# phd3/presto-1

Measured on AMD Instinct MI355X. Metric: probe_rows_per_sec, higher is better.
Workload: dtype int64+f64

## Files before the change

### presto-1_amd/__init__.py

```python
from . import _lib, expressions, operators, spi
from ._lib import SO_PATH, TgpuError, build
from .expressions import (and_, between, call, cast, coalesce, constant, field, if_, is_null, not_, or_)
from .operators import (ASC_NULLS_FIRST, ASC_NULLS_LAST, DESC_NULLS_FIRST, DESC_NULLS_LAST, DynamicFilterSourceOperatorFactory, MergePagesOperatorFactory, OrderByOperatorFactory, PartitionedOutputOperator, PartitionedOutputOperatorFactory, TopNOperatorFactory, AVG_BIGINT, AVG_DOUBLE, MIN_BIGINT, MAX_BIGINT, MIN_DOUBLE, MAX_DOUBLE, SUM_ORDER_EXACT, SUM_ORDER_JAVA, COUNT_ALL, COUNT_COLUMN, FINAL, FULL_OUTER, INNER, LOOKUP_OUTER, PARTIAL, PROBE_OUTER, SINGLE, SUM_BIGINT, SUM_DOUBLE,
                        Context, FilterAndProjectOperatorFactory, ScanFilterAndProjectOperatorFactory, PageSource, RecordCursor, FilterProjectHashAggregationOperatorFactory, FilterProjectLookupJoinOperatorFactory, GroupByHash, HashAggregationOperatorFactory, HashBuilderOperatorFactory,
                        LookupJoinOperatorFactory, LookupOuterOperatorFactory, Operator, OperatorFactory, page_processor_source, fused_probe_launch_counts, precompile_fused_aggregation, precompile_fused_probe, precompile_page_processor, to_pages,
                        SET_BITMAP, SET_GENERIC, SET_HASH, HashSemiJoinOperatorFactory, SetBuilderOperatorFactory, SetSupplier,
                        DistinctLimitOperatorFactory, MarkDistinctOperatorFactory,
                        LimitOperatorFactory, RowNumberOperatorFactory,
                        DENSE_RANK, RANK, ROW_NUMBER, TopNRankingOperatorFactory,
                        FRAME_PARTITION, FRAME_RANGE_TO_CURRENT, FRAME_ROWS_TO_CURRENT, WINDOW_AGGREGATE, WINDOW_CUME_DIST, WINDOW_DENSE_RANK, WINDOW_FIRST_VALUE,
                        WINDOW_LAG, WINDOW_LAST_VALUE, WINDOW_LEAD, WINDOW_PERCENT_RANK, WINDOW_RANK, WINDOW_ROW_NUMBER, WindowFunction, WindowOperatorFactory,
                        WINDOW_NTH_VALUE, WINDOW_NTILE, FRAME_TYPE_RANGE, FRAME_TYPE_ROWS, FRAME_TYPE_GROUPS, BOUND_UNBOUNDED_PRECEDING, BOUND_PRECEDING, BOUND_CURRENT_ROW,
                        BOUND_FOLLOWING, BOUND_UNBOUNDED_FOLLOWING, WindowFrame)
from .spi import (BIGINT, BOOLEAN, DATE, DOUBLE, INTEGER, VARCHAR, Block, DeviceBlock, DictionaryBlock, LazyBlock, OutputPage, Page, RunLengthEncodedBlock)
```

### presto-1_amd/_lib.py

```python
import ctypes as C
import os
import subprocess

_HERE = os.path.dirname(os.path.abspath(__file__))
SO_PATH = os.path.join(_HERE, "libtgpu.so")
CSRC = os.path.join(_HERE, "csrc")


class TgpuError(RuntimeError):

    NAMES = {-1: "INVALID_ARGUMENT", -2: "NUMERIC_VALUE_OUT_OF_RANGE", -3: "GENERIC_INSUFFICIENT_RESOURCES", -4: "COMPILER_ERROR",
             -5: "GENERIC_INTERNAL_ERROR", -6: "DEVICE_ERROR", -7: "DIVISION_BY_ZERO", -8: "NOT_SUPPORTED", -9: "INVALID_CAST_ARGUMENT"}

    def __init__(self, code, message):
        super().__init__(f"{self.NAMES.get(code, code)}: {message}")
        self.code = code
        self.message = message


def build(force=False, jobs=8):
    args = ["make", "-C", CSRC, f"-j{jobs}"]
    if force:
        args.append("-B")
    subprocess.check_call(args, stdout=subprocess.DEVNULL)
# ... 66 lines not shown
class WindowFrameSpec(C.Structure):
    _fields_ = [("type", C.c_int32), ("start_type", C.c_int32), ("start_channel", C.c_int32), ("end_type", C.c_int32), ("end_channel", C.c_int32)]


_lib = None

i32, i64, vp, cp = C.c_int32, C.c_int64, C.c_void_p, C.c_char_p
P = C.POINTER
SYMBOLS = {
    "tgpu_context_create": (i32, [i32, vp, P(vp)]),
    "tgpu_context_destroy": (None, [vp]),
    "tgpu_context_synchronize": (i32, [vp]),
    "tgpu_last_error": (cp, []),
    "tgpu_version": (cp, []),
    "tgpu_fused_probe_launch_counts": (i32, [P(i64)]),
    "tgpu_set_resource_dir": (i32, [cp]),
    "tgpu_context_set_double_sum_order": (i32, [vp, i32]),
    "tgpu_context_set_device_input_stable": (i32, [vp, i32]),
    "tgpu_orc_decode_long_column": (i32, [vp, i32, i32, i32, vp, i64, vp, i64, vp]),
    "tgpu_orc_decode_boolean_column": (i32, [vp, i32, vp, i64, vp, i64, vp]),
    "tgpu_orc_decode_dictionary_string_column": (i32, [vp, i32, i32, vp, i64, vp, i64, i32, vp, i64, vp, i64, vp]),
    "tgpu_orc_decode_direct_string_column": (i32, [vp, i32, i32, vp, i64, vp, i64, vp, i64, vp]),
    "tgpu_orc_decode_double_column": (i32, [vp, i32, vp, i64, vp, i64, vp]),
    "tgpu_parquet_decode_data_page": (i32, [vp, i32, i32, i32, i32, vp, i64, vp, i64, vp, i64, i32, vp]),
    "tgpu_context_set_max_output_page": (i32, [vp, i64, i64]),
    "tgpu_pinned_alloc": (i32, [vp, i64, P(vp)]),
    "tgpu_pinned_free": (i32, [vp, vp]),
    "tgpu_profile_enable": (i32, [vp, i32]),
    "tgpu_profile_reset": (i32, [vp]),
    "tgpu_profile_dump": (i64, [vp, cp, i64]),
# ... 118 lines not shown
```

### presto-1_amd/csrc/c_api.cpp

```cpp
#include <atomic>
#include <cstdlib>
#include <map>
#include <mutex>

#include "exchange.h"
#include "kernels.h"
#include "operators.h"
#include "serde.h"
#include "orc.h"
#include "parquet.h"

namespace tgpu {
const std::string &last_error();
}

using namespace tgpu;

namespace {

template <typename F> int32_t guard(F &&f)
{
    try {
        f();
        return TGPU_OK;
// ... 123 lines not shown
int32_t tgpu_context_synchronize(tgpu_context *ctx)
{
    return guard_on(ctx_of(ctx), [&] {
        TG_CHECK_ARG(ctx != nullptr, "context is null");
        ctx->ctx->sync();
    });
}

const char *tgpu_last_error(void) { return last_error().c_str(); }
long long tgpu_debug_bind_count(void) { return g_bind_count.load(); }
const char *tgpu_version(void) { return "tgpu 0.1 (gfx950)"; }
int32_t tgpu_fused_probe_launch_counts(int64_t out[3])
{
    if (!out) return TGPU_ERR_INVALID_ARGUMENT;
    tgpu::fused_probe_launch_counts(out);
    return TGPU_OK;
}

int32_t tgpu_set_resource_dir(const char *dir)
{
    return guard([&] {
        TG_CHECK_ARG(dir != nullptr, "dir is null");
        set_resource_dir(dir);
    });
}

int32_t tgpu_context_set_max_output_page(tgpu_context *ctx, int64_t max_bytes, int64_t max_rows)
{
    return guard_on(ctx_of(ctx), [&] {
        TG_CHECK_ARG(ctx != nullptr && max_bytes >= 0 && max_rows >= 0, "bad argument");
// ... 1320 lines not shown
```

### presto-1_amd/csrc/jit.cpp

```cpp
#include "jit.h"

#include <dlfcn.h>
#include <hip/hiprtc.h>
#include <sys/stat.h>
#include <unistd.h>

#include <algorithm>
#include <fstream>
#include <functional>
#include <list>
#include <tuple>
#include <set>
#include <sstream>

#include "agg.h"
#include "groupby.h"
#include "join.h"
#include "kernels.h"

namespace tgpu {

static std::string g_resource_dir;
static std::mutex g_jit_mu;

// ... 865 lines not shown
    for (int32_t i = 0; i < spec->node_count; i++) {
        const tgpu_expr_node &n = spec->nodes[i];
        put_i32(k, n.kind); put_i32(k, n.type); put_i32(k, n.op); put_i32(k, n.n_args);
        put_i32(k, n.args[0]); put_i32(k, n.args[1]); put_i32(k, n.args[2]); put_i32(k, n.is_null);
        put_i64(k, n.ival);
        k.append(reinterpret_cast<const char *>(&n.dval), 8);
        put_i32(k, n.slen);
    }
    put_i32(k, spec->string_pool_len);
    if (spec->string_pool && spec->string_pool_len > 0) k.append(spec->string_pool, (size_t)spec->string_pool_len);
    put_i32(k, spec->filter_root);
    put_i32(k, spec->projection_count);
    for (int32_t i = 0; i < spec->projection_count; i++) put_i32(k, spec->projection_roots[i]);
    put_i32(k, (int32_t)extra.size());
    for (int32_t v : extra) put_i32(k, v);
    for (const char *env : {"TGPU_FG_EXP", "TGPU_FJ_EXP", "TGPU_FA_STRIPES", "TGPU_FJ_STRIPES", "TGPU_FG_STRIPES"}) {
        const char *v = getenv(env);
        k += '|';
        if (v) k += v;
    }
    return k;
}

template <typename T, typename Make> std::shared_ptr<T> cached_object(const std::string &key, Make make)
{
    static LruCache<T> objects(jit_cache_capacity());
    return objects.get(key, make);
}
}

std::shared_ptr<PageProcessorGpu> PageProcessorGpu::shared(const std::vector<int32_t> &input_types, const tgpu_page_processor_spec *spec)
// ... 152 lines not shown
  void* carry[4];           // FJ_CARRY: block-private regions of the probe-side output VALUES (pass 1 evaluates them from its row
  unsigned char* carry_nulls; // registers for every emitted pair; pass 2 moves them instead of re-reading the input columns sparsely)
  unsigned long long* host_out; // epilogue (small pages): host-visible result words, written by the LAST workgroup of pass 1 (null: none)
  unsigned int* done;           //                         workgroups that have finished (rests at 0)
  const FpArgs* pages;          // FJ_EPILOGUE == 2 (a launch over a LIST of pages): one FpArgs per page, in device memory
  const int* page_tile0;        //   first tile of each page in the launch's tile sequence, [n_pages] = all tiles
  int n_pages;
  int pad3;
};
#define FJ_STRIPES @FJ_STRIPES@
#define FJ_TILE (FJ_STRIPES * 256)
#define FJ_COUNT_SLOTS 64
#ifndef FJ_EPILOGUE
#define FJ_EPILOGUE 0   // the variant for pages (few, one-tile chunks): pass 1 ends with the scan and hands its totals to the host itself
#endif

// rows-capacity offset of block b's private pair region: CHUNKS of 2^chunk_shift consecutive tiles are dealt round-robin, block b
// owns ceil((chunks - b) / grid) of them
__device__ inline long long fj_region_base(long long b, long long tiles, long long grid, int chunk_shift) {
  const long long chunks = (tiles + (1LL << chunk_shift) - 1) >> chunk_shift;
  const long long q = chunks / grid, r = chunks % grid;
  return ((b * q + (b < r ? b : r)) << chunk_shift) * FJ_TILE;
}

@CARRY_FUNCS@
// pass 1: one lane per row.  Matches are compacted in input order inside the tile (ballot + popcount) and appended to the
// block's PRIVATE region, so workgroups never communicate; a scan over the per-tile counts (in tile = input order) then
// gives every tile its final offset and pass 2 moves the pairs there -- probe positions come out ascending exactly as
// LookupJoinPageBuilder.java:144-153 requires.
//
// A probe is a chain of three dependent loads (row -> pre-filter word -> table slot).  The loop is software-pipelined over
// the block's tiles so that the three kinds of load of one iteration belong to three different tiles and are issued back to
// back: iteration `it` issues the row loads of tile it, the pre-filter loads of tile it-1, the slot loads of tile it-2 and
// compacts / writes the pairs of tile it-3, whose slots arrived during the previous iteration.  One memory round trip per
// iteration instead of three (vmcnt is in-order on CDNA: a wait for a dependent load would also wait for every prefetch
// issued before it, so "prefetch, then probe" inside one iteration cannot overlap).
__device__ __forceinline__ void fj_probe_body(const FjArgs& J, const unsigned int bid, const unsigned int nblk) {
  const FpArgs& A = J.fp;
  const int lane = threadIdx.x & 63, w = threadIdx.x >> 6;
  __shared__ int C[2][4];   // pairs of each wave, double-buffered by tile parity (one barrier per tile)
  const long long region = fj_region_base(bid, J.tiles, nblk, J.chunk_shift);
  long long local = 0;      // pairs this block has written so far (uniform across the block)
  unsigned int selected = 0;   // per lane: rows that passed the filter (a lane sees fewer than 2^31 rows)
  // Row layout of a tile: wave w owns the contiguous rows [w * 64 * FJ_STRIPES, (w + 1) * 64 * FJ_STRIPES) of the tile and its
  // lane reads row s * 64 + lane of them in stripe s (512 contiguous bytes per wave and load).  Input order inside the tile is
  // then (wave, stripe, lane): the compaction needs the other waves' TOTALS only, everything else is wave-local scalar work.
  // Rows are 32-bit here (a page has fewer than 2^31 positions).
#if FJ_EPILOGUE != 2
  const unsigned int n_rows = (unsigned int)A.n;
#endif
  const unsigned int wave_row = (unsigned int)w * (64u * FJ_STRIPES) + (unsigned int)lane;
// ... 14 lines not shown
  // the descriptor of the page stage A will load from is fetched ONE ITERATION AHEAD (scalar loads: the search of the tile's page and the
  // page's column pointers are two dependent round trips that would otherwise sit in front of every iteration's row loads)
  int pN = 0;
  long long tN = 0;   // tile of the next iteration's stage A (my_tiles == 0: unused)
  {
    const long long t0 = tile_of(0);
    tN = (my_tiles > 0 && t0 < J.tiles) ? t0 : 0;
    while (tN >= (long long)pt0[pN + 1]) pN++;
  }
  FpArgs AN = pgs[pN];    // next stage A's page
  FpArgs AB = AN;         // this iteration's stage B page (= the previous iteration's stage A page)
  long long tB0 = 0;      // first tile of that page
  long long tN0 = pt0[pN];
#endif
  long long chunk_local0 = 0;   // `local` at the start of the chunk being compacted
  TgRow rw[FJ_STRIPES];                                                                                            // stage A -> B
  long long pkey[FJ_STRIPES]; unsigned int psidx[FJ_STRIPES]; unsigned long long pbw[FJ_STRIPES];                      // B -> C
#if FJ_PF == 2
  unsigned long long pbits[FJ_STRIPES];     // Bloom mask of the key
#else
  unsigned int pbits[FJ_STRIPES];           // bit of the key inside its bitmap word
#endif
  unsigned char pfl[FJ_STRIPES];                                                                                   // 1 = probe, 2 = passed the filter
#if FJ_PF == 1 || FJ_PF == 3
  const unsigned long long key_range = (unsigned long long)J.pf.key_max - (unsigned long long)J.pf.key_min;
#endif
  long long skey[FJ_STRIPES]; unsigned int ssidx[FJ_STRIPES]; unsigned char sfl[FJ_STRIPES]; TgSlot16 ssl[FJ_STRIPES]; // C -> D
#if FJ_CARRY
  TgOut pov[FJ_STRIPES], sov[FJ_STRIPES];   // the row's output values, travelling B -> C -> D with its key
#pragma unroll
  for (int s = 0; s < FJ_STRIPES; s++) { tg_zero_out(pov[s]); tg_zero_out(sov[s]); }
#endif
#if FJ_CARRY == 2
  // PARTIAL carry: only outputs that the filter / key row already holds travel (no load, no TgRow field is added), and stage D keeps
  // its place behind the loads -- the values of tile jD step aside (dov) before stage C takes the stage registers for tile jC
  TgOut dov[FJ_STRIPES];
#pragma unroll
  for (int s = 0; s < FJ_STRIPES; s++) tg_zero_out(dov[s]);
#endif
#pragma unroll
  for (int s = 0; s < FJ_STRIPES; s++) {
    tg_zero_row(rw[s]);
    pkey[s] = 0; psidx[s] = 0; pbits[s] = 0; pbw[s] = 0; pfl[s] = 0;
    skey[s] = 0; ssidx[s] = 0; sfl[s] = 0; ssl[s].key = 0; ssl[s].head = -1; ssl[s].count = 0;
  }
  for (long long it = 0; it < my_tiles + 3; it++) {
    const long long jD = it - 3, jC = it - 2, jB = it - 1, jA = it;
    __builtin_amdgcn_s_waitcnt(0x0F70);   // vmcnt(0): everything the previous iteration issued (consumed right below anyway)
    // stage D, part 1: resolve tile jD from the slots loaded by the previous iteration; only a collision with another key
    // walks further
    int head[FJ_STRIPES];
    bool emit[FJ_STRIPES];
#pragma unroll
    for (int s = 0; s < FJ_STRIPES; s++) { head[s] = -1; emit[s] = false; }
    const bool doD = jD >= 0 && tile_of(jD) < J.tiles;
    if (doD) {
#pragma unroll
      for (int s = 0; s < FJ_STRIPES; s++) {
#if FJ_PF == 3
        // the bitmap is exact: the key is in the build side.  The pair carries the key's rank among the build keys (present keys
        // in front of its bitmap word, loaded by the previous iteration, + set bits below its own); fj_emit reads the build
        // position at that rank, for the matching rows only
        // (nobody reads the build positions: the rank structure may not even be built -- rank_base[0] is then whatever the buffer held)
// ... 110 lines not shown
#pragma unroll
    for (int s = 0; s < FJ_STRIPES; s++) bidx[s] = 0;
    if (doB) {
#if FJ_EPILOGUE == 2
      const unsigned int n_rows = (unsigned int)AB.n;
      const unsigned int row0 = (unsigned int)((tile_of(jB) - tB0) * FJ_TILE) + wave_row;   // the page's own rows
#else
      const FpArgs& AB = A;
      const unsigned int row0 = (unsigned int)(tile_of(jB) * FJ_TILE) + wave_row;
#endif
#pragma unroll
      for (int s = 0; s < FJ_STRIPES; s++) {
        const unsigned int row = row0 + s * 64;
        bool sel = false, passed = false;
        long long key = 0;
        if (row < n_rows && tg_filter(AB, row, rw[s])) {
          selected++;
          passed = true;
          const bool kn = tg_key(AB, row, rw[s], key);   // JoinProbe.java:87-97: a null probe key never matches
          sel = !kn;
#if FJ_CARRY
          tg_carry_eval(AB, row, rw[s], pov[s]);
#endif
        }
        bidx[s] = 0;
#if FJ_PF == 1 || FJ_PF == 3
        {
          // key in [key_min, key_max] <=> (key - key_min) mod 2^64 <= key_max - key_min; a key outside cannot match: no probe
          const unsigned long long d = (unsigned long long)key - (unsigned long long)J.pf.key_min;
          sel = sel && d <= key_range;
          pbits[s] = (unsigned int)d & 63u;
          bidx[s] = sel ? (unsigned int)(d >> 6) : 0u;
        }
#elif FJ_PF == 2
        {
          const unsigned long long hm = tg_fmix64((unsigned long long)tg_hash_long(key));
          pbits[s] = tg_bloom_mask(hm);
// ... 21 lines not shown
      ssl[s].head = J.pf.rank_base[cidx[s]];   // DIRECT layout: present keys in front of the survivor's bitmap word (entry 0 otherwise: unused)
#else
      ssl[s] = J.slots[cidx[s]];
#endif
    }
#pragma unroll
    for (int s = 0; s < FJ_STRIPES; s++) {
#if FJ_PF == 1 || FJ_PF == 3
      pbw[s] = J.pf.bitmap[bidx[s]];
#elif FJ_PF == 2
      pbw[s] = J.pf.bloom[bidx[s]];
#else
      pbw[s] = ~0ULL;
#endif
    }
    {
#if FJ_EPILOGUE == 2
      // this iteration's page was fetched by the previous one (idle stage: the same page again, its first tile)
      const FpArgs AA = AN;
      const long long tA = doA ? tN : tN0;
      const unsigned int n_rows = (unsigned int)AA.n;
      const unsigned int tile_row0 = (unsigned int)((tA - tN0) * FJ_TILE);
      const unsigned int row0 = tile_row0 + wave_row;
      AB = AA;      // (stage B of the NEXT iteration works on the rows loaded here; this iteration's stage B has run already)
      tB0 = tN0;
      {             // and the page of the next iteration's tile: issued now, needed in an iteration's time
        const long long jn = jA + 1;
        if (jn < my_tiles && tile_of(jn) < J.tiles) {
          tN = tile_of(jn);
          while (tN >= (long long)pt0[pN + 1]) pN++;
          tN0 = pt0[pN];
          AN = pgs[pN];
        }
      }
#else
      const FpArgs& AA = A;
      const unsigned int row0 = (unsigned int)((doA ? tile_of(jA) : 0LL) * FJ_TILE) + wave_row;
      const unsigned int tile_row0 = (unsigned int)((doA ? tile_of(jA) : 0LL) * FJ_TILE);
#endif
      if (tile_row0 + FJ_TILE <= n_rows) {   // interior tile: one address per column, the stripes are constant offsets from it
#pragma unroll
        for (int s = 0; s < FJ_STRIPES; s++) tg_load_row(AA, row0 + s * 64, rw[s]);
      }
      else {
#pragma unroll
        for (int s = 0; s < FJ_STRIPES; s++) {
          const unsigned int row = row0 + s * 64;
          tg_load_row(AA, row < n_rows ? row : n_rows - 1, rw[s]);
        }
      }
    }
    __builtin_amdgcn_sched_barrier(0);
#if FJ_CARRY != 1
    // stage D, part 2: compact the pairs of tile jD in input order and append them to the block's region
    if (doD) {
      const long long tile = tile_of(jD);
      const unsigned int row0 = (unsigned int)(tile * FJ_TILE) + wave_row;
      if ((jD & cmask) == 0) chunk_local0 = local;
      unsigned long long b[FJ_STRIPES];
      int wave_total = 0;
#pragma unroll
      for (int s = 0; s < FJ_STRIPES; s++) {
        b[s] = __ballot(emit[s]);
        wave_total += __popcll(b[s]);
      }
      int* Cw = C[jD & 1];
      if (lane == 0) Cw[w] = wave_total;
// ... 16 lines not shown
        }
        o += (unsigned int)__popcll(b[s]);
      }
      local += tile_total;
      // per-chunk bookkeeping, rewritten after every tile of the chunk (the last one stands)
      if (threadIdx.x == 0) {
#if FJ_EPILOGUE   // (agent-scope store: the epilogue's reader may sit on another XCD)
        __hip_atomic_store(&J.tile_cnt[tile >> csh], (int)(local - chunk_local0), __ATOMIC_RELAXED, __HIP_MEMORY_SCOPE_AGENT);
#else
        J.tile_cnt[tile >> csh] = (int)(local - chunk_local0);
#endif
        J.tile_src[tile >> csh] = (int)chunk_local0;
      }
    }
#endif
  }
  // rows that passed the filter: ONE atomic per workgroup, spread over FJ_COUNT_SLOTS words on separate cache lines (the host adds
  unsigned long long selected_wave = selected;
#pragma unroll
  for (int d = 32; d >= 1; d >>= 1) selected_wave += __shfl_down(selected_wave, d, 64);
  __shared__ unsigned long long S[4];
  if (lane == 0) S[w] = selected_wave;
  __syncthreads();
#if !FJ_EPILOGUE
  if (threadIdx.x == 0) {
    const unsigned long long block_total = S[0] + S[1] + S[2] + S[3];
    if (block_total) atomicAdd(&J.counters[(bid % FJ_COUNT_SLOTS) * 16], block_total);
  }
}
#else
  // Epilogue of a small page (J.host_out): the workgroup that finishes LAST scans the chunk counts into the chunks' output offsets (what
// ... 180 lines not shown
        if (nd.kind == TGPU_EX_CALL || nd.kind == TGPU_EX_SPECIAL)
            for (int k = 0; k < nd.n_args; k++)
                if (can_raise(nd.args[k])) return true;
        return false;
    };
    for (size_t ch = 0; ch < proj_roots_.size(); ch++)
        if ((int)ch != join_channel_ && can_raise(proj_roots_[ch])) supported_ = false;
    key_can_raise_ = can_raise(proj_roots_[(size_t)join_channel_]);
    if (supported_) generate();
}

FusedProbeGpu::~FusedProbeGpu() {}

static std::atomic<int64_t> g_fj_launches[3];
constexpr int kFjFreeRule = 1;
void fused_probe_launch_counts(int64_t out[3])
{
    for (int i = 0; i < 3; i++) out[i] = g_fj_launches[i].load(std::memory_order_relaxed);
}

void FusedProbeGpu::generate()
{
    auto cols_decl = [&](const Gen &g) {
        std::ostringstream cols;
        for (int ch : g.used_cols) {
            const int32_t t = input_types_[(size_t)ch];
            const char *T = (t == TGPU_VARCHAR || t == TGPU_BOOLEAN) ? "unsigned char" : ctype(t);
            cols << "  const " << T << "* c" << ch << " = (const " << T << "*)A.col_values[" << ch << "]; (void)c" << ch << ";\n";
            cols << "  const unsigned char* cn" << ch << " = FJ_NO_NULLS ? (const unsigned char*)0 : A.col_nulls[" << ch << "]; (void)cn" << ch << ";\n";
            if (t == TGPU_VARCHAR) cols << "  const int* co" << ch << " = A.col_offsets[" << ch << "]; (void)co" << ch << ";\n";
        }
        return cols.str();
    };
// ... 92 lines not shown
    src << "#if FJ_CARRY\n";
    for (int ch : carry_only_cols) src << field(ch);
    src << "#endif\n";
    if (gr.reg_cols.empty()) src << "  int unused;\n";
    src << "};\n__device__ inline void tg_load_row(const FpArgs& A, long long row, TgRow& R) {\n";
    for (int ch : gr.reg_cols) src << load(ch);
    src << "#if FJ_CARRY\n";
    for (int ch : carry_only_cols) src << load(ch);
    src << "#endif\n";
    src << "  (void)A; (void)row; (void)R;\n}\n__device__ inline void tg_zero_row(TgRow& R) {\n";
    for (int ch : gr.reg_cols) src << "  R.c" << ch << " = 0; R.n" << ch << " = 0;\n";
    src << "#if FJ_CARRY\n";
    for (int ch : carry_only_cols) src << "  R.c" << ch << " = 0; R.n" << ch << " = 0;\n";
    src << "#endif\n";
    src << "  (void)R;\n}\n";
    const std::string rc = cols_decl(gr), mc = cols_decl(gm);
    for (auto &b : reg_bodies) src << splice(b, rc);
    for (auto &b : mem_bodies) src << splice(b, mc);
    src << "struct FjArgs;\nstruct TgOut {\n";
    for (size_t i = 0; i < output_channels_.size(); i++) src << all_or_free(i) << "  " << ctype(proj_types_[(size_t)output_channels_[i]]) << " v" << i << ";\n#endif\n";
    src << "#if !FJ_NO_NULLS\n  unsigned char nulls;\n#endif\n};\n__device__ inline void tg_zero_out(TgOut& O) {\n";
    for (size_t i = 0; i < output_channels_.size(); i++) src << all_or_free(i) << "  O.v" << i << " = 0;\n#endif\n";
    src << "#if !FJ_NO_NULLS\n  O.nulls = 0;\n#endif\n  (void)O;\n}\n#if FJ_CARRY\n";
    {
        const std::string cc = cols_decl(gc);
        for (size_t i = 0; i < carry_bodies.size(); i++) src << all_or_free(i) << splice(carry_bodies[i], cc) << "#endif\n";
        src << "__device__ inline void tg_carry_eval(const FpArgs& A, long long row, const TgRow& R, TgOut& O) {\n  unsigned char nl = 0;\n";
        for (size_t i = 0; i < output_channels_.size(); i++) {
            const int32_t t = proj_types_[(size_t)output_channels_[i]];
            src << all_or_free(i) << "  { " << ctype(t) << " v = 0; const bool n = tg_c" << i << "(A, row, R, v); O.v" << i << " = n ? (" << ctype(t) << ")0 : v; nl |= n ? " << (1 << i)
// ... 19 lines not shown
                    << "]) A.out_nulls[" << i << "][to] = (unsigned char)((nl >> " << i << ") & 1u);\n#endif\n";
    }
    carry_funcs << "}\n#endif\n";
    (void)kt;
    src << "__device__ inline void tg_emit_outputs(const FpArgs& A, long long row, long long o) {\n  (void)A; (void)row; (void)o;\n";
    for (size_t i = 0; i < output_channels_.size(); i++) {
        const int ch = output_channels_[i];
        const int32_t t = proj_types_[(size_t)ch];
        const char *T = t == TGPU_BOOLEAN ? "unsigned char" : ctype(t);
        src << not_carried(i) << "  { " << ctype(t) << " v = 0; const bool n = tg_p" << ch << "(A, row, v); ((" << T << "*)A.out_values[" << i << "])[o] = n ? (" << T << ")0 : (" << T
            << ")v; if (A.out_nulls[" << i << "]) A.out_nulls[" << i << "][o] = n ? 1 : 0; }\n#endif\n";
    }
    src << "}\n";
    if (const char *exp = getenv("TGPU_FJ_EXP")) src << "#define FJ_EXP_" << exp << " 1\n";
    {
        std::string kernels = kFjKernels;
        const std::string tag = "@FJ_STRIPES@";
        kernels.replace(kernels.find(tag), tag.size(), std::to_string(fj_stripes()));
        const std::string ctag = "@CARRY_FUNCS@";
        kernels.replace(kernels.find(ctag), ctag.size(), carry_funcs.str());
        src << kernels;
    }
    source_ = src.str();
}

static std::string prefilter_source(const std::string &src, int variant)
{
    static const char *layout[4] = {"plain", "bitmap", "bloom", "direct"};
    const std::string l = layout[variant % 4];
    return "#define FJ_PF " + std::to_string(variant % 4) + "\n#define FJ_NO_NULLS " + std::to_string((variant / 4) % 2) + "\n#define FJ_CARRY " + std::to_string(variant / 24) +
           "\n#define FJ_EPILOGUE " + std::to_string((variant / 8) % 3) + "\n#define fj_pair fj_pair_" + l + "\n#define fj_probe fj_probe_" + l +
           "\n#define fj_emit fj_emit_" + l + "\n" + src;
}

void FusedProbeGpu::precompile()
{
    if (!supported_) return;
    for (int variant = 0; variant < 24; variant++) {
        (void)code_object_for(prefilter_source(source_, variant));
        if (partial_supported_ && (variant % 4 == 1 || variant % 4 == 3) && variant / 8 < 2) (void)code_object_for(prefilter_source(source_, 48 + variant));
    }
}

JitModule *FusedProbeGpu::module_for(int kind, bool no_nulls, int carry, int epilogue)
{
    std::lock_guard<std::mutex> lk(mu_);
    const int variant = kind + (no_nulls ? 4 : 0) + epilogue * 8 + carry * 24;
    if (!modules_[variant]) modules_[variant] = load_module(prefilter_source(source_, variant));
    return modules_[variant].get();
}

struct FusedProbeGpu::Pending {
    FjArgs J{};
    JitModule *module = nullptr;
    int pf_kind = 0;
    int64_t chunks = 0;
    bool outer = false, need_build_positions = false;
    int carry = 0;
    BufferPtr tile_cnt, tile_src, tile_dst, misc, pair_probe, pair_build;
    std::vector<BufferPtr> carry_regions;
    Context::AsyncRead read;
    Context::Signal signal;
// ... 47 lines not shown
    int64_t n = in.n;
    if (multi) {
        int64_t t = 0;
        for (const DevicePage *pg : pages) {
            TG_CHECK_ARG(pg->n > 0, "empty page in a multi-page launch");
            page_tile0.push_back((int32_t)t);
            t += ceil_div(pg->n, tile_rows);
        }
        page_tile0.push_back((int32_t)t);
        TG_CHECK_ARG(t <= kFjMultiMaxTiles, "too many rows for one multi-page launch");
        n = t * tile_rows;
        carry = 0;
    }
    if (n == 0) return nullptr;
    const bool page_variant = multi || (ceil_div(n, tile_rows) <= kFjEpilogueMaxChunks && getenv("TGPU_DISABLE_PROBE_EPILOGUE") == nullptr);
    JitModule *module = module_for(tv.rank_base ? 3 : (tv.bitmap ? 1 : (tv.bloom ? 2 : 0)), !any_nulls, carry, multi ? 2 : (page_variant ? 1 : 0));
    std::shared_ptr<Pending> pend = std::make_shared<Pending>();
    pend->col_nulls = col_nulls;
    pend->kernel_variant = multi ? 2 : (page_variant ? 1 : 0);
    if (page_variant) pend->signal = ctx->begin_signal();
    if (multi && pend->signal.slot < 0) return nullptr;
    struct SignalGuard {
        Context *ctx;
        Context::Signal *signal;
        bool armed = true;
        ~SignalGuard()
        {
            if (armed && signal->slot >= 0) {
                ctx->abandon_signal(*signal);
                signal->slot = -1;
            }
// ... 12 lines not shown
    J.fp.n = multi ? in.n : n;
    J.slots = tv.slots;
    J.mask = tv.mask;
    J.bitmap = tv.bitmap;
    J.key_min = tv.key_min;
    J.key_max = tv.key_max;
    J.bloom = tv.bloom;
    J.bloom_word_mask = tv.bloom_word_mask;
    J.direct = tv.direct;
    J.rank_base = tv.rank_base;
    J.outer = (outer ? 1 : 0) | (need_build_positions ? 0 : 2);
    J.tiles = ceil_div(n, tile_rows);
    TG_CHECK_ARG(n <= 0x7fffffffLL && J.tiles <= 0x7fffffffLL, "page too large");
    const int pf_kind = tv.rank_base ? 3 : (tv.bitmap ? 1 : (tv.bloom ? 2 : 0));
    static const char *probe_names[4] = {"fj_probe_plain", "fj_probe_bitmap", "fj_probe_bloom", "fj_probe_direct"};
    const int64_t resident = (int64_t)ctx->cu_count() * module->blocks_per_cu(probe_names[pf_kind]);
    int chunk_shift = 0;
    const int max_chunk_shift = getenv("TGPU_FJ_CHUNK_SHIFT") ? atoi(getenv("TGPU_FJ_CHUNK_SHIFT")) : 6;
    while (!multi && chunk_shift < max_chunk_shift && (J.tiles >> (chunk_shift + 1)) >= 4 * resident) chunk_shift++;
    J.chunk_shift = chunk_shift;
    const int64_t chunks = (J.tiles + (1ll << chunk_shift) - 1) >> chunk_shift;
    pend->chunks = chunks;
    pend->pf_kind = pf_kind;
    const int64_t grid1 = std::min<int64_t>(chunks, resident);
    J.grid1 = grid1;
    BufferPtr tile_cnt = ctx->alloc((size_t)chunks * 4), tile_src = ctx->alloc((size_t)chunks * 4), tile_dst = ctx->alloc((size_t)chunks * 4);
    constexpr int kMiscWords = kFjMiscWords;
    static_assert((size_t)kFjMiscWords * 8 <= Context::kZeroedScratchBytes, "the probe's counters fit the context's scratch words");
    if (pend->signal.slot >= 0 && chunk_shift != 0) {
        ctx->abandon_signal(pend->signal);
        pend->signal.slot = -1;
// ... 46 lines not shown
        for (size_t i = 0; i < output_channels_.size(); i++) {
            if (carry == 2 && !free_out_[i]) continue;
            carry_regions.push_back(ctx->alloc((size_t)cap * type_width(proj_types_[(size_t)output_channels_[i]])));
            J.carry[i] = carry_regions.back()->ptr();
            const tgpu_expr_node &root = nodes_[(size_t)proj_roots_[(size_t)output_channels_[i]]];
            nullable = nullable || !(root.kind == TGPU_EX_INPUT && root.op >= 0 && root.op < (int)in.cols.size() && in.cols[(size_t)root.op].nulls == nullptr);
        }
        if (nullable) {
            carry_regions.push_back(ctx->alloc((size_t)cap));
            J.carry_nulls = carry_regions.back()->as<uint8_t>();
        }
    }
    pend->grid1 = grid1;
    pend->tile_cnt = tile_cnt; pend->tile_src = tile_src; pend->tile_dst = tile_dst; pend->misc = misc; pend->pair_probe = pair_probe; pend->pair_build = pair_build;
    g_fj_launches[carry].fetch_add(1, std::memory_order_relaxed);
    if (launch || !epilogue) launch_probe(ctx, pend);
    signal_guard.armed = false;
    return pend;
}

void FusedProbeGpu::launch_probe(Context *ctx, const std::shared_ptr<Pending> &pend)
{
    static const char *probe_names[4] = {"fj_probe_plain", "fj_probe_bitmap", "fj_probe_bloom", "fj_probe_direct"};
    if (!pend || pend->probe_launched) return;
    FjArgs &J = pend->J;
    {
        ProfileScope ps(ctx, "fused_filter_probe");
        launch_args(pend->module->fn(probe_names[pend->pf_kind]), (int)pend->grid1, J, ctx->stream());
    }
    pend->probe_launched = true;
// ... 1481 lines not shown
```

### presto-1_amd/csrc/jit.h

```cpp
#pragma once

#include <algorithm>

#include "common.h"

namespace tgpu {

constexpr int kFpMaxCols = 24;
constexpr int kFpMaxProj = 16;

struct FpArgs {
    const void *col_values[kFpMaxCols];
    const uint8_t *col_nulls[kFpMaxCols];
    const int32_t *col_offsets[kFpMaxCols];
    void *out_values[kFpMaxProj];
    uint8_t *out_nulls[kFpMaxProj];
    int32_t *positions;
    const int32_t *tile_offsets;
    int32_t *tile_counts;
    unsigned long long *error;
    long long n;
    unsigned long long *sel_mask;
};

// ... 83 lines not shown
    void *carry[4];
    uint8_t *carry_nulls;
    unsigned long long *host_out;
    unsigned int *done;
    const FpArgs *pages;
    const int32_t *page_tile0;
    int32_t n_pages;
    int32_t pad3;
};
constexpr int kFjMaxBuildCols = 4;
constexpr int64_t kFjMultiMaxTiles = 32768;
constexpr int64_t kFjEpilogueMaxChunks = 2048;

class LookupSourceGpu;
void fused_probe_launch_counts(int64_t out[3]);

class FusedProbeGpu {
public:
    FusedProbeGpu(std::vector<int32_t> input_types, const tgpu_page_processor_spec *spec, int32_t join_channel, std::vector<int32_t> output_channels);
    ~FusedProbeGpu();
    static std::shared_ptr<FusedProbeGpu> shared(const std::vector<int32_t> &input_types, const tgpu_page_processor_spec *spec, int32_t join_channel,
                                                 const std::vector<int32_t> &output_channels);
    void precompile();
    bool supported() const { return supported_; }
    const std::vector<int32_t> &projection_types() const { return proj_types_; }
    void process(Context *ctx, const DevicePage &in, const LookupSourceGpu &source, bool outer, bool need_build_positions, std::vector<DeviceColumn> &probe_out,
                 BufferPtr &build_idx, int64_t &count, int64_t &selected_rows, const std::vector<DeviceColumn> *build_cols = nullptr,
                 std::vector<DeviceColumn> *build_out = nullptr);
    struct Pending;
    std::shared_ptr<Pending> begin(Context *ctx, const DevicePage &in, const LookupSourceGpu &source, bool outer, bool need_build_positions, bool launch = true);
    std::shared_ptr<Pending> begin(Context *ctx, const std::vector<const DevicePage *> &pages, const LookupSourceGpu &source, bool outer, bool need_build_positions,
                                   bool launch = true);
    static int64_t multi_page_row_limit();
    void finish(Context *ctx, const std::shared_ptr<Pending> &pending, const DevicePage &in, std::vector<DeviceColumn> &probe_out, BufferPtr &build_idx, int64_t &count,
                int64_t &selected_rows, const std::vector<DeviceColumn> *build_cols = nullptr, std::vector<DeviceColumn> *build_out = nullptr, bool launch = true);
    void launch_probe(Context *ctx, const std::shared_ptr<Pending> &pending);
    void launch_emit(Context *ctx, const std::shared_ptr<Pending> &pending);
    bool can_pair(const std::shared_ptr<Pending> &emit_side, const std::shared_ptr<Pending> &probe_side) const;
    void launch_pair(Context *ctx, const std::shared_ptr<Pending> &emit_side, const std::shared_ptr<Pending> &probe_side);
    void cancel(Context *ctx, const std::shared_ptr<Pending> &pending);
    const std::string &source() const { return source_; }

private:
    void generate();
    struct JitModule *module_for(int prefilter_kind, bool no_nulls, int carry, int epilogue);
    std::mutex mu_;
    std::vector<int32_t> input_types_;
    std::vector<tgpu_expr_node> nodes_;
    std::string pool_;
    int filter_root_;
    std::vector<int32_t> proj_roots_, proj_types_, output_channels_;
    int32_t join_channel_;
    bool supported_ = false;
    std::string source_;
    std::shared_ptr<JitModule> modules_[72];
    bool carry_supported_ = false;
    bool partial_supported_ = false, key_can_raise_ = false;
    std::vector<bool> free_out_;
};

class GroupedAccumulators;

class FusedAggGpu {
public:
    FusedAggGpu(std::vector<int32_t> input_types, const tgpu_page_processor_spec *spec, std::vector<tgpu_agg_spec> aggs,
                std::vector<int32_t> group_by_channels = {});
    static std::shared_ptr<FusedAggGpu> shared(const std::vector<int32_t> &input_types, const tgpu_page_processor_spec *spec,
                                               const std::vector<tgpu_agg_spec> &aggs, const std::vector<int32_t> &group_by_channels);
    const std::vector<int> &key_inputs() const { return key_inputs_; }
    void probe_groups(Context *ctx, const DevicePage &in, const struct GbhProbeLaunch &l);
// ... 51 lines not shown
```

### presto-1_amd/operators.py

```python
import ctypes as C
import json

import numpy as np

from . import _lib
from .expressions import FlatProgram
from .spi import OutputPage, Page

COUNT_ALL, COUNT_COLUMN, SUM_BIGINT, SUM_DOUBLE, AVG_BIGINT, AVG_DOUBLE, MIN_BIGINT, MAX_BIGINT, MIN_DOUBLE, MAX_DOUBLE = 1, 2, 3, 4, 5, 6, 7, 8, 9, 10
SINGLE, PARTIAL, FINAL = 0, 1, 2
ASC_NULLS_FIRST, ASC_NULLS_LAST, DESC_NULLS_FIRST, DESC_NULLS_LAST = 0, 1, 2, 3
INNER, PROBE_OUTER, LOOKUP_OUTER, FULL_OUTER = 0, 1, 2, 3
SUM_ORDER_EXACT, SUM_ORDER_JAVA = 0, 1


def _i32(seq):
    seq = list(seq)
    return (C.c_int32 * max(1, len(seq)))(*seq), len(seq)


class Context:

    def __init__(self, device=0, stream=None):
        h = C.c_void_p()
# ... 501 lines not shown
    gc, ng = _i32(group_by_channels)
    _lib.check(_lib.lib().tgpu_precompile_fused_aggregation(nt, t, C.byref(spec), len(aggs), arr, ng, gc))


def precompile_fused_probe(input_types, filter_expr, projections, join_channel, probe_output_channels):
    prog = FlatProgram(filter_expr, projections)
    spec, keep = prog.to_c()
    t, nt = _i32(input_types)
    oc, no = _i32(probe_output_channels)
    _lib.check(_lib.lib().tgpu_precompile_fused_probe(nt, t, C.byref(spec), join_channel, no, oc))


def fused_probe_launch_counts():
    out = (C.c_int64 * 3)()
    _lib.check(_lib.lib().tgpu_fused_probe_launch_counts(out))
    return tuple(int(v) for v in out)


class GroupByHash:

    def __init__(self, ctx: Context, types, hash_channels, input_hash_channel=None, expected_size=100):
        t, n = _i32(types)
        hc, _ = _i32(hash_channels)
        h = C.c_void_p()
        _lib.check(_lib.lib().tgpu_group_by_hash_create(ctx.handle, n, t, hc, -1 if input_hash_channel is None else input_hash_channel,
                                                        expected_size, C.byref(h)))
        self.handle = h

    def addPage(self, page: Page):
        cp, keep = page.to_c()
# ... 339 lines not shown
```

Before: 88.21 billion.

## Add depth-2 row prefetch to fused probe kernel with partial vmcnt wait

Adds a second set of row registers to the whole-table fused join probe kernel so the rows of the next tile are loaded while the current iteration waits for hash look-ups. The loop body is emitted twice per trip with alternating register sets, and the top-of-iteration wait leaves the youngest row loads outstanding using a computed vmcnt. Depth 2 is the default for carry modes 0 and 2 on whole-table launches, and it doubles the module variant table. In exchange it raises register pressure, which may lower occupancy, and increases JIT compile variants. Also adds depth launch counters and an env cap on resident blocks.

```diff
diff --git a/presto-1_amd/__init__.py b/presto-1_amd/__init__.py
--- a/presto-1_amd/__init__.py
+++ b/presto-1_amd/__init__.py
@@ -3,7 +3,7 @@
 from .expressions import (and_, between, call, cast, coalesce, constant, field, if_, is_null, not_, or_)
 from .operators import (ASC_NULLS_FIRST, ASC_NULLS_LAST, DESC_NULLS_FIRST, DESC_NULLS_LAST, DynamicFilterSourceOperatorFactory, MergePagesOperatorFactory, OrderByOperatorFactory, PartitionedOutputOperator, PartitionedOutputOperatorFactory, TopNOperatorFactory, AVG_BIGINT, AVG_DOUBLE, MIN_BIGINT, MAX_BIGINT, MIN_DOUBLE, MAX_DOUBLE, SUM_ORDER_EXACT, SUM_ORDER_JAVA, COUNT_ALL, COUNT_COLUMN, FINAL, FULL_OUTER, INNER, LOOKUP_OUTER, PARTIAL, PROBE_OUTER, SINGLE, SUM_BIGINT, SUM_DOUBLE,
                         Context, FilterAndProjectOperatorFactory, ScanFilterAndProjectOperatorFactory, PageSource, RecordCursor, FilterProjectHashAggregationOperatorFactory, FilterProjectLookupJoinOperatorFactory, GroupByHash, HashAggregationOperatorFactory, HashBuilderOperatorFactory,
-                        LookupJoinOperatorFactory, LookupOuterOperatorFactory, Operator, OperatorFactory, page_processor_source, fused_probe_launch_counts, precompile_fused_aggregation, precompile_fused_probe, precompile_page_processor, to_pages,
+                        LookupJoinOperatorFactory, LookupOuterOperatorFactory, Operator, OperatorFactory, page_processor_source, fused_probe_launch_counts, fused_probe_depth_counts, precompile_fused_aggregation, precompile_fused_probe, precompile_page_processor, to_pages,
                         SET_BITMAP, SET_GENERIC, SET_HASH, HashSemiJoinOperatorFactory, SetBuilderOperatorFactory, SetSupplier,
                         DistinctLimitOperatorFactory, MarkDistinctOperatorFactory,
                         LimitOperatorFactory, RowNumberOperatorFactory,
diff --git a/presto-1_amd/_lib.py b/presto-1_amd/_lib.py
--- a/presto-1_amd/_lib.py
+++ b/presto-1_amd/_lib.py
@@ -104,6 +104,7 @@
     "tgpu_last_error": (cp, []),
     "tgpu_version": (cp, []),
     "tgpu_fused_probe_launch_counts": (i32, [P(i64)]),
+    "tgpu_fused_probe_depth_counts": (i32, [P(i64)]),
     "tgpu_set_resource_dir": (i32, [cp]),
     "tgpu_context_set_double_sum_order": (i32, [vp, i32]),
     "tgpu_context_set_device_input_stable": (i32, [vp, i32]),
diff --git a/presto-1_amd/csrc/c_api.cpp b/presto-1_amd/csrc/c_api.cpp
--- a/presto-1_amd/csrc/c_api.cpp
+++ b/presto-1_amd/csrc/c_api.cpp
@@ -161,6 +161,12 @@
 {
     if (!out) return TGPU_ERR_INVALID_ARGUMENT;
     tgpu::fused_probe_launch_counts(out);
+    return TGPU_OK;
+}
+int32_t tgpu_fused_probe_depth_counts(int64_t out[2])
+{
+    if (!out) return TGPU_ERR_INVALID_ARGUMENT;
+    tgpu::fused_probe_depth_counts(out);
     return TGPU_OK;
 }
 
diff --git a/presto-1_amd/csrc/jit.cpp b/presto-1_amd/csrc/jit.cpp
--- a/presto-1_amd/csrc/jit.cpp
+++ b/presto-1_amd/csrc/jit.cpp
@@ -903,7 +903,7 @@
     for (int32_t i = 0; i < spec->projection_count; i++) put_i32(k, spec->projection_roots[i]);
     put_i32(k, (int32_t)extra.size());
     for (int32_t v : extra) put_i32(k, v);
-    for (const char *env : {"TGPU_FG_EXP", "TGPU_FJ_EXP", "TGPU_FA_STRIPES", "TGPU_FJ_STRIPES", "TGPU_FG_STRIPES"}) {
+    for (const char *env : {"TGPU_FG_EXP", "TGPU_FJ_EXP", "TGPU_FA_STRIPES", "TGPU_FJ_STRIPES", "TGPU_FG_STRIPES", "TGPU_FJ_DEPTH"}) {
         const char *v = getenv(env);
         k += '|';
         if (v) k += v;
@@ -1086,6 +1086,22 @@
 #ifndef FJ_EPILOGUE
 #define FJ_EPILOGUE 0   // the variant for pages (few, one-tile chunks): pass 1 ends with the scan and hands its totals to the host itself
 #endif
+#ifndef FJ_DEPTH
+#define FJ_DEPTH 1      // row sets in flight: 2 = the rows of the tile after next are loaded while this iteration's look-ups are waited for
+#endif
+#if FJ_DEPTH == 2 && FJ_EPILOGUE
+#error "FJ_DEPTH 2 is a variant of the whole-table kernel only"
+#endif
+#if FJ_DEPTH == 2
+// The iteration's wait leaves the youngest row set outstanding: vmcnt counts loads AND stores on this target and retires them in order,
+// so the row loads are the last vector-memory operations an iteration issues (behind the pair stores).  FJ_ROW_LOADS = load instructions
+// per row as generated; the count is 6 bits wide, [3:0] and [15:14] of the operand (0x0F70: no wait on the other counters).  Correctness
+// does not rest on the number: the compiler adds whatever wait a register use needs.
+#define FJ_PENDING (FJ_ROW_LOADS * FJ_STRIPES > 63 ? 63 : FJ_ROW_LOADS * FJ_STRIPES)
+#define FJ_WAIT (0x0F70 | (FJ_PENDING & 15) | ((FJ_PENDING >> 4) << 14))
+#else
+#define FJ_WAIT 0x0F70  // vmcnt(0): everything the previous iteration issued (consumed right below anyway)
+#endif
 
 // rows-capacity offset of block b's private pair region: CHUNKS of 2^chunk_shift consecutive tiles are dealt round-robin, block b
 // owns ceil((chunks - b) / grid) of them
@@ -1107,6 +1123,12 @@
 // compacts / writes the pairs of tile it-3, whose slots arrived during the previous iteration.  One memory round trip per
 // iteration instead of three (vmcnt is in-order on CDNA: a wait for a dependent load would also wait for every prefetch
 // issued before it, so "prefetch, then probe" inside one iteration cannot overlap).
+//
+// FJ_DEPTH 2 (whole-table launches): a second set of row registers.  Iteration `it` issues the rows of tile it+1 -- as its LAST
+// vector-memory operations, behind the pair stores -- and waits at its top for everything but that youngest set, so a wave always has a
+// tile's rows in flight, also while it waits for its look-ups.  Stage B of iteration `it` consumes the set issued by iteration it-2 (tile
+// it-1; the prologue issues tile 0).  The two sets alternate by writing the loop body twice per trip, never by copying registers (a copy
+// from a register with a pending load waits for the load).  Rows per lane, compaction order and pairs are those of depth 1.
 __device__ __forceinline__ void fj_probe_body(const FjArgs& J, const unsigned int bid, const unsigned int nblk) {
   const FpArgs& A = J.fp;
   const int lane = threadIdx.x & 63, w = threadIdx.x >> 6;
@@ -1151,7 +1173,11 @@
   long long tN0 = pt0[pN];
 #endif
   long long chunk_local0 = 0;   // `local` at the start of the chunk being compacted
+#if FJ_DEPTH == 2
+  TgRow rwa[FJ_STRIPES], rwb[FJ_STRIPES];                                                                          // stage A -> B: tiles of even / odd j
+#else
   TgRow rw[FJ_STRIPES];                                                                                            // stage A -> B
+#endif
   long long pkey[FJ_STRIPES]; unsigned int psidx[FJ_STRIPES]; unsigned long long pbw[FJ_STRIPES];                      // B -> C
 #if FJ_PF == 2
   unsigned long long pbits[FJ_STRIPES];     // Bloom mask of the key
@@ -1177,13 +1203,27 @@
 #endif
 #pragma unroll
   for (int s = 0; s < FJ_STRIPES; s++) {
+#if FJ_DEPTH == 2
+    tg_zero_row(rwa[s]); tg_zero_row(rwb[s]);
+#else
     tg_zero_row(rw[s]);
+#endif
     pkey[s] = 0; psidx[s] = 0; pbits[s] = 0; pbw[s] = 0; pfl[s] = 0;
     skey[s] = 0; ssidx[s] = 0; sfl[s] = 0; ssl[s].key = 0; ssl[s].head = -1; ssl[s].count = 0;
   }
-  for (long long it = 0; it < my_tiles + 3; it++) {
-    const long long jD = it - 3, jC = it - 2, jB = it - 1, jA = it;
-    __builtin_amdgcn_s_waitcnt(0x0F70);   // vmcnt(0): everything the previous iteration issued (consumed right below anyway)
+#if FJ_DEPTH == 2
+  // whole trips of two iterations: an exit between the two instances of the body would be one more way into the loop header for the compiler's
+  // wait-count bookkeeping, with the other row set pending there.  The odd iteration out is idle (every tile at or past my_tiles is past J.tiles).
+  const long long n_it = (my_tiles + 4) & ~1LL;
+#else
+  const long long n_it = my_tiles + 3;
+#endif
+@FJ_LOOP@
+)SRC";
+
+const char *kFjLoopBody = R"SRC(
+    const long long jD = it - 3, jC = it - 2, jB = it - 1, jA = it + (FJ_DEPTH - 1);
+    __builtin_amdgcn_s_waitcnt(FJ_WAIT);
     // stage D, part 1: resolve tile jD from the slots loaded by the previous iteration; only a collision with another key
     // walks further
     int head[FJ_STRIPES];
@@ -1324,13 +1364,13 @@
         const unsigned int row = row0 + s * 64;
         bool sel = false, passed = false;
         long long key = 0;
-        if (row < n_rows && tg_filter(AB, row, rw[s])) {
+        if (row < n_rows && tg_filter(AB, row, @RW@[s])) {
           selected++;
           passed = true;
-          const bool kn = tg_key(AB, row, rw[s], key);   // JoinProbe.java:87-97: a null probe key never matches
+          const bool kn = tg_key(AB, row, @RW@[s], key);   // JoinProbe.java:87-97: a null probe key never matches
           sel = !kn;
 #if FJ_CARRY
-          tg_carry_eval(AB, row, rw[s], pov[s]);
+          tg_carry_eval(AB, row, @RW@[s], pov[s]);
 #endif
         }
         bidx[s] = 0;
@@ -1382,6 +1422,20 @@
       pbw[s] = ~0ULL;
 #endif
     }
+#if FJ_DEPTH != 2
+@ROW_LOADS@
+#endif
+    __builtin_amdgcn_sched_barrier(0);
+@STAGE_D2@
+#if FJ_DEPTH == 2
+    // the rows of tile jA = it + 1: the youngest vector-memory operations of the iteration, behind stage D's stores (see FJ_WAIT)
+    __builtin_amdgcn_sched_barrier(0);
+@ROW_LOADS@
+    __builtin_amdgcn_sched_barrier(0);
+#endif
+)SRC";
+
+const char *kFjRowLoads = R"SRC(
     {
 #if FJ_EPILOGUE == 2
       // this iteration's page was fetched by the previous one (idle stage: the same page again, its first tile)
@@ -1408,17 +1462,19 @@
 #endif
       if (tile_row0 + FJ_TILE <= n_rows) {   // interior tile: one address per column, the stripes are constant offsets from it
 #pragma unroll
-        for (int s = 0; s < FJ_STRIPES; s++) tg_load_row(AA, row0 + s * 64, rw[s]);
+        for (int s = 0; s < FJ_STRIPES; s++) tg_load_row(AA, row0 + s * 64, @RW@[s]);
       }
       else {
 #pragma unroll
         for (int s = 0; s < FJ_STRIPES; s++) {
           const unsigned int row = row0 + s * 64;
-          tg_load_row(AA, row < n_rows ? row : n_rows - 1, rw[s]);
+          tg_load_row(AA, row < n_rows ? row : n_rows - 1, @RW@[s]);
         }
       }
     }
-    __builtin_amdgcn_sched_barrier(0);
+)SRC";
+
+const char *kFjStageD2 = R"SRC(
 #if FJ_CARRY != 1
     // stage D, part 2: compact the pairs of tile jD in input order and append them to the block's region
     if (doD) {
@@ -1465,7 +1521,9 @@
       }
     }
 #endif
-  }
+)SRC";
+
+const char *kFjKernelsTail = R"SRC(
   // rows that passed the filter: ONE atomic per workgroup, spread over FJ_COUNT_SLOTS words on separate cache lines (the host adds
   unsigned long long selected_wave = selected;
 #pragma unroll
@@ -1676,9 +1734,21 @@
 
 static std::atomic<int64_t> g_fj_launches[3];
 constexpr int kFjFreeRule = 1;
+static std::atomic<int64_t> g_fj_depth_launches[2];
+constexpr int kFjDepthByCarry[3] = {2, 1, 2};
+static int fj_depth_for(int carry, int epilogue)
+{
+    if (epilogue != 0) return 1;
+    if (const char *e = getenv("TGPU_FJ_DEPTH")) return atoi(e) == 2 ? 2 : 1;
+    return kFjDepthByCarry[carry];
+}
 void fused_probe_launch_counts(int64_t out[3])
 {
     for (int i = 0; i < 3; i++) out[i] = g_fj_launches[i].load(std::memory_order_relaxed);
+}
+void fused_probe_depth_counts(int64_t out[2])
+{
+    for (int i = 0; i < 2; i++) out[i] = g_fj_depth_launches[i].load(std::memory_order_relaxed);
 }
 
 void FusedProbeGpu::generate()
@@ -1801,6 +1871,7 @@
     for (int ch : carry_only_cols) src << "  R.c" << ch << " = 0; R.n" << ch << " = 0;\n";
     src << "#endif\n";
     src << "  (void)R;\n}\n";
+    src << "#define FJ_ROW_LOADS ((" << gr.reg_cols.size() << " + (FJ_CARRY == 1 ? " << carry_only_cols.size() << " : 0)) * (FJ_NO_NULLS ? 1 : 2))\n";
     const std::string rc = cols_decl(gr), mc = cols_decl(gm);
     for (auto &b : reg_bodies) src << splice(b, rc);
     for (auto &b : mem_bodies) src << splice(b, mc);
@@ -1850,7 +1921,16 @@
     src << "}\n";
     if (const char *exp = getenv("TGPU_FJ_EXP")) src << "#define FJ_EXP_" << exp << " 1\n";
     {
-        std::string kernels = kFjKernels;
+        auto replace_all = [](std::string t, const std::string &tag, const std::string &with) {
+            for (size_t p = t.find(tag); p != std::string::npos; p = t.find(tag, p + with.size())) t.replace(p, tag.size(), with);
+            return t;
+        };
+        const std::string body = replace_all(replace_all(kFjLoopBody, "@STAGE_D2@", kFjStageD2), "@ROW_LOADS@", kFjRowLoads);
+        const std::string loop = std::string("#if FJ_DEPTH == 2\n  {\n    const long long jA = 0;\n    const bool doA = jA < my_tiles && tile_of(jA) < J.tiles;\n") +
+                                 replace_all(kFjRowLoads, "@RW@", "rwa") + "  }\n  for (long long it = 0; it < n_it;) {\n    {\n" + replace_all(body, "@RW@", "rwb") +
+                                 "    }\n    ++it;\n    {\n" + replace_all(body, "@RW@", "rwa") + "    }\n    ++it;\n  }\n#else\n" +
+                                 "  for (long long it = 0; it < n_it; it++) {\n" + replace_all(body, "@RW@", "rw") + "  }\n#endif\n";
+        std::string kernels = replace_all(kFjKernels, "@FJ_LOOP@", loop) + kFjKernelsTail;
         const std::string tag = "@FJ_STRIPES@";
         kernels.replace(kernels.find(tag), tag.size(), std::to_string(fj_stripes()));
         const std::string ctag = "@CARRY_FUNCS@";
@@ -1864,8 +1944,8 @@
 {
     static const char *layout[4] = {"plain", "bitmap", "bloom", "direct"};
     const std::string l = layout[variant % 4];
-    return "#define FJ_PF " + std::to_string(variant % 4) + "\n#define FJ_NO_NULLS " + std::to_string((variant / 4) % 2) + "\n#define FJ_CARRY " + std::to_string(variant / 24) +
-           "\n#define FJ_EPILOGUE " + std::to_string((variant / 8) % 3) + "\n#define fj_pair fj_pair_" + l + "\n#define fj_probe fj_probe_" + l +
+    return "#define FJ_PF " + std::to_string(variant % 4) + "\n#define FJ_NO_NULLS " + std::to_string((variant / 4) % 2) + "\n#define FJ_CARRY " + std::to_string((variant / 24) % 3) +
+           "\n#define FJ_DEPTH " + std::to_string(variant / 72 + 1) + "\n#define FJ_EPILOGUE " + std::to_string((variant / 8) % 3) + "\n#define fj_pair fj_pair_" + l + "\n#define fj_probe fj_probe_" + l +
            "\n#define fj_emit fj_emit_" + l + "\n" + src;
 }
 
@@ -1873,15 +1953,17 @@
 {
     if (!supported_) return;
     for (int variant = 0; variant < 24; variant++) {
-        (void)code_object_for(prefilter_source(source_, variant));
-        if (partial_supported_ && (variant % 4 == 1 || variant % 4 == 3) && variant / 8 < 2) (void)code_object_for(prefilter_source(source_, 48 + variant));
-    }
-}
-
-JitModule *FusedProbeGpu::module_for(int kind, bool no_nulls, int carry, int epilogue)
+        const int epilogue = variant / 8;
+        (void)code_object_for(prefilter_source(source_, variant + 72 * (fj_depth_for(0, epilogue) - 1)));
+        if (partial_supported_ && (variant % 4 == 1 || variant % 4 == 3) && epilogue < 2)
+            (void)code_object_for(prefilter_source(source_, 48 + variant + 72 * (fj_depth_for(2, epilogue) - 1)));
+    }
+}
+
+JitModule *FusedProbeGpu::module_for(int kind, bool no_nulls, int carry, int epilogue, int depth)
 {
     std::lock_guard<std::mutex> lk(mu_);
-    const int variant = kind + (no_nulls ? 4 : 0) + epilogue * 8 + carry * 24;
+    const int variant = kind + (no_nulls ? 4 : 0) + epilogue * 8 + carry * 24 + (depth - 1) * 72;
     if (!modules_[variant]) modules_[variant] = load_module(prefilter_source(source_, variant));
     return modules_[variant].get();
 }
@@ -1959,7 +2041,8 @@
     }
     if (n == 0) return nullptr;
     const bool page_variant = multi || (ceil_div(n, tile_rows) <= kFjEpilogueMaxChunks && getenv("TGPU_DISABLE_PROBE_EPILOGUE") == nullptr);
-    JitModule *module = module_for(tv.rank_base ? 3 : (tv.bitmap ? 1 : (tv.bloom ? 2 : 0)), !any_nulls, carry, multi ? 2 : (page_variant ? 1 : 0));
+    const int depth = fj_depth_for(carry, multi ? 2 : (page_variant ? 1 : 0));
+    JitModule *module = module_for(tv.rank_base ? 3 : (tv.bitmap ? 1 : (tv.bloom ? 2 : 0)), !any_nulls, carry, multi ? 2 : (page_variant ? 1 : 0), depth);
     std::shared_ptr<Pending> pend = std::make_shared<Pending>();
     pend->col_nulls = col_nulls;
     pend->kernel_variant = multi ? 2 : (page_variant ? 1 : 0);
@@ -2002,7 +2085,8 @@
     TG_CHECK_ARG(n <= 0x7fffffffLL && J.tiles <= 0x7fffffffLL, "page too large");
     const int pf_kind = tv.rank_base ? 3 : (tv.bitmap ? 1 : (tv.bloom ? 2 : 0));
     static const char *probe_names[4] = {"fj_probe_plain", "fj_probe_bitmap", "fj_probe_bloom", "fj_probe_direct"};
-    const int64_t resident = (int64_t)ctx->cu_count() * module->blocks_per_cu(probe_names[pf_kind]);
+    int64_t resident = (int64_t)ctx->cu_count() * module->blocks_per_cu(probe_names[pf_kind]);
+    if (const char *cap = getenv("TGPU_FJ_MAX_BLOCKS")) resident = std::min<int64_t>(resident, std::max(1, atoi(cap)));
     int chunk_shift = 0;
     const int max_chunk_shift = getenv("TGPU_FJ_CHUNK_SHIFT") ? atoi(getenv("TGPU_FJ_CHUNK_SHIFT")) : 6;
     while (!multi && chunk_shift < max_chunk_shift && (J.tiles >> (chunk_shift + 1)) >= 4 * resident) chunk_shift++;
@@ -2079,6 +2163,7 @@
     pend->grid1 = grid1;
     pend->tile_cnt = tile_cnt; pend->tile_src = tile_src; pend->tile_dst = tile_dst; pend->misc = misc; pend->pair_probe = pair_probe; pend->pair_build = pair_build;
     g_fj_launches[carry].fetch_add(1, std::memory_order_relaxed);
+    g_fj_depth_launches[depth - 1].fetch_add(1, std::memory_order_relaxed);
     if (launch || !epilogue) launch_probe(ctx, pend);
     signal_guard.armed = false;
     return pend;
diff --git a/presto-1_amd/csrc/jit.h b/presto-1_amd/csrc/jit.h
--- a/presto-1_amd/csrc/jit.h
+++ b/presto-1_amd/csrc/jit.h
@@ -121,6 +121,7 @@
 
 class LookupSourceGpu;
 void fused_probe_launch_counts(int64_t out[3]);
+void fused_probe_depth_counts(int64_t out[2]);
 
 class FusedProbeGpu {
 public:
@@ -150,7 +151,7 @@
 
 private:
     void generate();
-    struct JitModule *module_for(int prefilter_kind, bool no_nulls, int carry, int epilogue);
+    struct JitModule *module_for(int prefilter_kind, bool no_nulls, int carry, int epilogue, int depth);
     std::mutex mu_;
     std::vector<int32_t> input_types_;
     std::vector<tgpu_expr_node> nodes_;
@@ -160,7 +161,7 @@
     int32_t join_channel_;
     bool supported_ = false;
     std::string source_;
-    std::shared_ptr<JitModule> modules_[72];
+    std::shared_ptr<JitModule> modules_[144];
     bool carry_supported_ = false;
     bool partial_supported_ = false, key_can_raise_ = false;
     std::vector<bool> free_out_;
diff --git a/presto-1_amd/operators.py b/presto-1_amd/operators.py
--- a/presto-1_amd/operators.py
+++ b/presto-1_amd/operators.py
@@ -539,6 +539,12 @@
 def fused_probe_launch_counts():
     out = (C.c_int64 * 3)()
     _lib.check(_lib.lib().tgpu_fused_probe_launch_counts(out))
+    return tuple(int(v) for v in out)
+
+
+def fused_probe_depth_counts():
+    out = (C.c_int64 * 2)()
+    _lib.check(_lib.lib().tgpu_fused_probe_depth_counts(out))
     return tuple(int(v) for v in out)
 
 
```

Result: faster. 92.52 billion, median of 6 (+4.9%).
